# YuHang-max/3DSAD-main

Measured on AMD Instinct MI355X. Metric: scenes/sec (16384-pt KITTI-shaped) through SA+cluster path, higher is better.
Workload: dtype f32

## Files before the change

### 3dsad-main_amd/csrc/mlp_layer.hip

```cpp
#include "common.h"
#include <map>
#include <mutex>
#include <utility>

namespace {

#include "reg_common.h"

constexpr int LWAVES = 4;
constexpr int SLOTS = 16;

using sad::LayerJob;
using sad::LayerMulti;

constexpr int KC = 2;
constexpr int STAGE_F4 = KC * 8 * 64;

__device__ __forceinline__ int job_rows(const LayerJob &jb) { return jb.rowtab ? jb.rowtab[0] : jb.rows; }

struct RowInfo {
    int q, grp;
    bool live, whole;
    unsigned xoff;
    float4 rel;
};
template <bool GATHER>
__device__ __forceinline__ RowInfo row_info(const LayerJob &jb, int rt, int lane, bool need_gid) {
    RowInfo r;
    const int j = lane & 31, h = lane >> 5;
    const int total = job_rows(jb);
    r.q = rt * 32 + j;
    r.live = r.q < total;
    if (!r.live) r.q = total - 1;
    int src = r.q, gv = 0;
    if (GATHER || need_gid) gv = jb.row_gid[r.q];
    if (GATHER) src = jb.row_src[r.q];
    r.grp = gv & (WHOLE_BIT - 1);
    r.whole = (gv & WHOLE_BIT) != 0;
    r.xoff = (unsigned)src * (unsigned)jb.ldx * 4u;
    r.rel = make_float4(0.f, 0.f, 0.f, 0.f);
    if (GATHER && h == 0) {
        const float *pq = jb.xyz + (long long)src * 3;
        const float *pc = jb.new_xyz + (long long)r.grp * 3;
        r.rel = make_float4(pq[0] - pc[0], pq[1] - pc[1], pq[2] - pc[2], 0.f);
    }
    return r;
}

struct Chunk { float4 a0, a1, a2, a3, b0, b1, b2, b3; };
static_assert(KC == 4 || KC == 2, "Chunk holds up to four activation fragments");

template <bool GATHER>
__device__ __forceinline__ Chunk load_chunk_of(const LayerJob &jb, const unsigned xoff, const int ob, const int c, const int wave, const int lane) {
    const int h = lane >> 5;
    const int KG = jb.kg;
    const char *xb = reinterpret_cast<const char *>(jb.x);
    const float4 *wf = reinterpret_cast<const float4 *>(jb.packed + jb.off + jb.np) + (size_t)(ob * 4) * KG * 64;
    const unsigned ulane = (unsigned)lane;
    float4 ga[4], gb[KC];
#pragma unroll
    for (int i = 0; i < KC; ++i) {
        const int f = wave * KC + i;
        const int gk = c * KC + (f >> 2);
        ga[i] = (wf + ((size_t)(f & 3) * KG + (gk < KG ? gk : KG - 1)) * 64)[ulane];
    }
#pragma unroll
    for (int u = 0; u < KC; ++u) {
        int g = c * KC + u;
        g = g < KG ? g : KG - 1;
        if constexpr (GATHER) {
            const int ch = 2 * g - 1 + h;
            const int cc = ch < 0 ? 0 : (ch < jb.cpr ? ch : jb.cpr - 1);
            gb[u] = *reinterpret_cast<const float4 *>(xb + (size_t)(xoff + 16u * (unsigned)cc));
        } else {
            gb[u] = *reinterpret_cast<const float4 *>((xb + (size_t)g * 32) + (size_t)(xoff + 16u * (unsigned)h));
        }
    }
    return Chunk{ga[0], ga[1], ga[KC > 2 ? 2 : 0], ga[KC > 2 ? 3 : 0], gb[0], gb[1], gb[KC > 2 ? 2 : 0], gb[KC > 2 ? 3 : 0]};
}

struct Prefetched {
    Chunk ck;
    float4 rel;
    unsigned xoff;
    int valid;
    int next;
};
struct NextItem {
    int ji;
    int rb, ob;
};
struct NextSource {
    int dyn;
    int pulled;
    int stat;
    int own;
};
constexpr int META_ITEM = 0, META_I0 = 1, META_N = 2;

template <bool GATHER, bool LAST>
__device__ __forceinline__ Prefetched gemm_item(const LayerMulti &lm, const LayerJob &jb, const int rb, const int ob, float4 *lds,
                                                const Prefetched pin, const NextSource ns) {
    Prefetched pre;
    pre.valid = 0;
    pre.next = 0x7FFFFFFF;
    int *meta = reinterpret_cast<int *>(lds + 2 * STAGE_F4);
    auto publish_next = [&]() {
        if (ns.dyn && threadIdx.x == 0) meta[META_ITEM] = ns.pulled * 8 + ns.own;
    };
    const int tid = threadIdx.x, lane = tid & 63, wave = __builtin_amdgcn_readfirstlane(tid >> 6);
    const int h = lane >> 5;
    const int wy = wave >> 1, wx = wave & 1;
    const int KG = jb.kg;
    const int NC = (KG + KC - 1) / KC;
    unsigned fr_xoff;
    float4 fr_rel;
    if (pin.valid) {
        fr_xoff = pin.xoff;
        fr_rel = pin.rel;
    } else {
        const RowInfo fr = row_info<GATHER>(jb, rb * 4 + wave, lane, false);
        fr_xoff = fr.xoff;
        fr_rel = fr.rel;
    }
    auto load_chunk = [&](int c) -> Chunk { return load_chunk_of<GATHER>(jb, fr_xoff, ob, c, wave, lane); };
    auto store_chunk = [&](const Chunk ck, int c, float4 *st) {
        const float4 ga[4] = {ck.a0, ck.a1, ck.a2, ck.a3}, gb[4] = {ck.b0, ck.b1, ck.b2, ck.b3};
#pragma unroll
        for (int i = 0; i < KC; ++i) {
            const int f = wave * KC + i;
            st[((f >> 2) * 8 + (f & 3)) * 64 + lane] = ga[i];
        }
#pragma unroll
        for (int u = 0; u < KC; ++u) {
            const int g = c * KC + u;
            float4 v = gb[u];
            if constexpr (GATHER) {
                const int ch = 2 * g - 1 + h;
                const bool ok = ch >= 0 && ch < jb.cpr;
                v.x = ok ? v.x : 0.f; v.y = ok ? v.y : 0.f; v.z = ok ? v.z : 0.f; v.w = ok ? v.w : 0.f;
                const bool first = g == 0 && h == 0;
                v.x = first ? fr_rel.x : v.x; v.y = first ? fr_rel.y : v.y; v.z = first ? fr_rel.z : v.z; v.w = first ? fr_rel.w : v.w;
            }
            if (g >= KG) v = make_float4(0.f, 0.f, 0.f, 0.f);
            float ops[4];
            to_operands(v.x, v.y, v.z, v.w, ops);
            st[(u * 8 + 4 + wave) * 64 + lane] = make_float4(ops[0], ops[1], ops[2], ops[3]);
        }
    };
    f32x16 acc[2][2];
    {
        const float *bias = jb.packed + jb.off + (ob * 4 + 2 * wx) * 32;
#pragma unroll
        for (int oc = 0; oc < 2; ++oc)
#pragma unroll
            for (int a = 0; a < 4; ++a) {
                const float4 bv = *reinterpret_cast<const float4 *>(bias + oc * 32 + 8 * a + 4 * h);
#pragma unroll
                for (int rt = 0; rt < 2; ++rt) {
                    acc[rt][oc][4 * a + 0] = bv.x; acc[rt][oc][4 * a + 1] = bv.y; acc[rt][oc][4 * a + 2] = bv.z; acc[rt][oc][4 * a + 3] = bv.w;
                }
            }
    }
    __syncthreads();
    Chunk nxt;
    if (pin.valid) nxt = pin.ck;
    else nxt = load_chunk(0);
    store_chunk(nxt, 0, lds);
    if (NC == 1) publish_next();
    __syncthreads();
#pragma unroll 1
    for (int c = 0; c < NC; ++c) {
        float4 *cur = lds + (c & 1) * STAGE_F4;
        if (c + 1 < NC) {
            nxt = load_chunk(c + 1);
        } else {
          const int nitem = __builtin_amdgcn_readfirstlane(ns.dyn ? meta[META_ITEM] : ns.stat);
          const int mi0 = __builtin_amdgcn_readfirstlane(meta[META_I0]);
          pre.next = nitem;
          if (nitem < __builtin_amdgcn_readfirstlane(meta[META_N])) {
            const int nji = nitem < mi0 ? 0 : 1;
            const int nit = nitem - (nji ? mi0 : 0);
            const int nnog = nji ? lm.j[1].nog : lm.j[0].nog;
            NextItem nx;
            nx.ji = nji;
            nx.rb = nit / nnog;
            nx.ob = nit % nnog;
#define SAD_FETCH_NEXT(NJ)                                                                         \
    do {                                                                                           \
        if ((NJ).gather) {                                                                         \
            const RowInfo nf = row_info<true>((NJ), nx.rb * 4 + wave, lane, false);                \
            pre.xoff = nf.xoff;                                                                    \
            pre.rel = nf.rel;                                                                      \
            pre.ck = load_chunk_of<true>((NJ), nf.xoff, nx.ob, 0, wave, lane);                     \
        } else {                                                                                   \
            const RowInfo nf = row_info<false>((NJ), nx.rb * 4 + wave, lane, false);               \
            pre.xoff = nf.xoff;                                                                    \
            pre.rel = nf.rel;                                                                      \
            pre.ck = load_chunk_of<false>((NJ), nf.xoff, nx.ob, 0, wave, lane);                    \
        }                                                                                          \
    } while (0)
            if (nx.ji == 0) SAD_FETCH_NEXT(lm.j[0]);
            else SAD_FETCH_NEXT(lm.j[1]);
#undef SAD_FETCH_NEXT
            pre.valid = 1;
          }
        }
        float4 wa[2][2], xa[2][2];
#pragma unroll
        for (int i = 0; i < 2; ++i) {
            wa[0][i] = cur[(0 * 8 + 2 * wx + i) * 64 + lane];
            xa[0][i] = cur[(0 * 8 + 4 + 2 * wy + i) * 64 + lane];
        }
#pragma unroll
        for (int u = 0; u < KC; ++u) {
            if (u + 1 < KC) {
#pragma unroll
                for (int i = 0; i < 2; ++i) {
                    wa[(u + 1) & 1][i] = cur[((u + 1) * 8 + 2 * wx + i) * 64 + lane];
                    xa[(u + 1) & 1][i] = cur[((u + 1) * 8 + 4 + 2 * wy + i) * 64 + lane];
                }
            }
            __builtin_amdgcn_sched_barrier(0);
#pragma unroll
            for (int rt = 0; rt < 2; ++rt) {
                const float ops[4] = {xa[u & 1][rt].x, xa[u & 1][rt].y, xa[u & 1][rt].z, xa[u & 1][rt].w};
#pragma unroll
                for (int oc = 0; oc < 2; ++oc) acc[rt][oc] = mma4(acc[rt][oc], wa[u & 1][oc], ops);
            }
            __builtin_amdgcn_sched_barrier(0);
        }
        if (c + 1 < NC) store_chunk(nxt, c + 1, lds + ((c + 1) & 1) * STAGE_F4);
        if (c + 2 == NC) publish_next();
        __syncthreads();
    }
    if (jb.relu) {
#pragma unroll
        for (int rt = 0; rt < 2; ++rt)
#pragma unroll
            for (int oc = 0; oc < 2; ++oc)
#pragma unroll
                for (int g = 0; g < 16; ++g) acc[rt][oc][g] = acc[rt][oc][g] > 0.f ? acc[rt][oc][g] : 0.f;
    }
#pragma unroll
    for (int rt = 0; rt < 2; ++rt) {
        const RowInfo ri = row_info<false>(jb, rb * 4 + 2 * wy + rt, lane, LAST);
        const int j = lane & 31;
        if constexpr (!LAST) {
            if (ri.live) {
                float *yrow = jb.y + (long long)ri.q * jb.ldy + (ob * 4 + 2 * wx) * 32 + 4 * h;
#pragma unroll
                for (int oc = 0; oc < 2; ++oc)
#pragma unroll
                    for (int a = 0; a < 4; ++a)
                        *reinterpret_cast<float4 *>(yrow + oc * 32 + 8 * a) =
                            make_float4(acc[rt][oc][4 * a], acc[rt][oc][4 * a + 1], acc[rt][oc][4 * a + 2], acc[rt][oc][4 * a + 3]);
            }
        } else {
            float *stage = reinterpret_cast<float *>(lds) + wave * (SLOTS * 64);
            const int key = ri.live ? ri.grp + 1 : 0;
            const PoolMasks pm = pool_masks(key);
            const int nkey = __shfl_down(key, 1, 64), pkey = __shfl_up(key, 1, 64);
            const bool tail = ri.live && (j == 31 || nkey != key);
            const bool head = ri.live && (j == 0 || pkey != key);
            const unsigned heads = (unsigned)__ballot(head), tails = (unsigned)__ballot(tail);
            const int ngroups = __builtin_popcount(heads);
            const int slot = __builtin_popcount(heads & (0xFFFFFFFFu >> (31 - j))) - 1;
            const bool staged = ngroups <= SLOTS;
            const int ch0 = (ob * 4 + 2 * wx) * 32;
#pragma unroll
            for (int oc = 0; oc < 2; ++oc) {
                const f32x16 t = seg_max16(acc[rt][oc], pm);
                if (!tail) continue;
                if (staged) {
                    float *d = stage + slot * 64 + oc * 32 + 4 * h;
#pragma unroll
                    for (int a = 0; a < 4; ++a) *reinterpret_cast<float4 *>(d + 8 * a) = make_float4(t[4 * a], t[4 * a + 1], t[4 * a + 2], t[4 * a + 3]);
                } else {
                    float *o = jb.out + (long long)ri.grp * jb.ld_out + jb.col_off + ch0 + oc * 32 + 4 * h;
#pragma unroll
                    for (int a = 0; a < 4; ++a)
#pragma unroll
                        for (int e = 0; e < 4; ++e) {
                            if (ch0 + oc * 32 + 8 * a + 4 * h + e >= jb.cout_last) continue;
                            if (ri.whole) o[8 * a + e] = t[4 * a + e];
                            else atomic_max_pos(o + 8 * a + e, t[4 * a + e]);
                        }
                }
            }
            if (staged) {
                unsigned rem = tails;
                for (int s = 0; s < ngroups; ++s) {
                    const int p = __builtin_ctz(rem);
                    rem &= rem - 1;
                    const int g = __builtin_amdgcn_readlane(ri.grp, p);
                    const bool w = __builtin_amdgcn_readlane((int)ri.whole, p) != 0;
                    float *orow = jb.out + (long long)g * jb.ld_out + jb.col_off + ch0;
                    const float *sp = stage + s * 64;
                    if (ch0 + lane < jb.cout_last) {
                        if (w) orow[lane] = sp[lane];
                        else atomic_max_pos(orow + lane, sp[lane]);
                    }
                }
            }
        }
    }
    return pre;
}

__global__ __launch_bounds__(LWAVES * 64) __attribute__((amdgpu_waves_per_eu(2, 2))) void mlp_layer_kernel(const LayerMulti lm) {
    extern __shared__ __attribute__((aligned(16))) float4 lds4[];
    int *meta = reinterpret_cast<int *>(lds4 + 2 * STAGE_F4);
    const int i0 = ((job_rows(lm.j[0]) + 127) / 128) * lm.j[0].nog;
    const int nitems = lm.n > 1 ? i0 + ((job_rows(lm.j[1]) + 127) / 128) * lm.j[1].nog : i0;
    const int dyn = lm.queue != nullptr;
    const sad::ItemQueue Q = sad::itemq_init(lm.queue, dyn ? 8 : 0);
    int item = blockIdx.x;
    if (threadIdx.x == 0) {
        meta[META_I0] = i0;
        meta[META_N] = nitems;
        if (dyn) meta[META_ITEM] = sad::itemq_item(Q, Q.own, sad::itemq_pull(Q));
    }
    __syncthreads();
    if (dyn) item = meta[META_ITEM];
    Prefetched pre;
    pre.valid = 0;
    while (true) {
        if (item >= nitems) {
            if (!dyn) break;
            __syncthreads();
            if (threadIdx.x == 0) meta[META_ITEM] = sad::itemq_steal(Q, nitems);
            __syncthreads();
            item = meta[META_ITEM];
            if (item >= nitems) break;
            pre.valid = 0;
        }
        const int ji = item < i0 ? 0 : 1;
        const int it = item - (ji ? i0 : 0);
        const LayerJob &jb = lm.j[ji];
        const int nog = jb.nog;
        NextSource ns;
        ns.dyn = dyn;
        ns.pulled = 0;
        if (dyn && threadIdx.x == 0) ns.pulled = sad::itemq_pull(Q);
        ns.stat = item + (int)gridDim.x;
        ns.own = Q.own;
        if (jb.gather) {
            if (jb.last) pre = gemm_item<true, true>(lm, jb, it / nog, it % nog, lds4, pre, ns);
            else pre = gemm_item<true, false>(lm, jb, it / nog, it % nog, lds4, pre, ns);
        } else {
            if (jb.last) pre = gemm_item<false, true>(lm, jb, it / nog, it % nog, lds4, pre, ns);
            else pre = gemm_item<false, false>(lm, jb, it / nog, it % nog, lds4, pre, ns);
        }
        item = pre.next;
    }
    if (dyn && threadIdx.x == 0) sad::itemq_done(Q, (int)gridDim.x);
}

}

namespace sad {

int *stream_item_queue(hipStream_t st) {
    static std::mutex mu;
    static std::map<std::pair<int, hipStream_t>, int *> queues;
    hipStreamCaptureStatus cap = hipStreamCaptureStatusNone;
    if (hipStreamIsCapturing(st, &cap) != hipSuccess || cap != hipStreamCaptureStatusNone) {
        (void)hipGetLastError();
        return nullptr;
    }
    int dev = 0;
    if (hipGetDevice(&dev) != hipSuccess) {
        (void)hipGetLastError();
        return nullptr;
    }
    std::lock_guard<std::mutex> lk(mu);
    auto it = queues.find({dev, st});
    if (it != queues.end()) return it->second;
    int *q = nullptr;
    if (hipMalloc(&q, sizeof(int) * ITEMQ_INTS) != hipSuccess) {
        (void)hipGetLastError();
        return nullptr;
    }
    if (hipMemsetAsync(q, 0, sizeof(int) * ITEMQ_INTS, st) != hipSuccess) {
        (void)hipGetLastError();
        (void)hipFree(q);
        return nullptr;
    }
    queues[{dev, st}] = q;
    return q;
}

int launch_layers(const LayerMulti &lm_in, long long max_items, hipStream_t st) {
    LayerMulti lm = lm_in;
    lm.queue = get_option(OPT_MLP_LAYER_QUEUE) == 1 ? stream_item_queue(st) : nullptr;
    static std::atomic<uint64_t> attr_done{0};
    lds_attr_once(attr_done, reinterpret_cast<const void *>(&mlp_layer_kernel), 160 * 1024);
    const size_t lds = sizeof(float4) * ((size_t)2 * STAGE_F4 + 1);
    static std::atomic<int> per_cu{0};
    int pc = per_cu.load(std::memory_order_relaxed);
    if (pc == 0) {
        int nb = 0;
        if (hipOccupancyMaxActiveBlocksPerMultiprocessor(&nb, mlp_layer_kernel, LWAVES * 64, lds) != hipSuccess || nb < 1) {
            (void)hipGetLastError();
            nb = 2;
        }
        pc = nb > 2 ? 2 : nb;
        per_cu.store(pc, std::memory_order_relaxed);
    }
    if (get_option(OPT_MLP_DYN_SLOTS) > 0 && get_option(OPT_MLP_DYN_SLOTS) < pc) pc = get_option(OPT_MLP_DYN_SLOTS);
    const int cus = sad::device_cus();
    long long grid = (long long)cus * pc;
    const long long cap = max_items;
    if (grid > cap) grid = cap < 1 ? 1 : cap;
    hipLaunchKernelGGL(mlp_layer_kernel, dim3((unsigned)grid), dim3(LWAVES * 64), lds, st, lm);
    return check_launch("sad_mlp_chain_f32 (layer-streamed chain)");
}

}
```

### 3dsad-main_amd/csrc/reg_common.h

```cpp
#pragma once
#include "prims.h"

constexpr int WHOLE_BIT = 1 << 30;
using sad::RegChain;
using sad::RegMulti;

struct Swapped { float lo, hi; };
__device__ __forceinline__ Swapped swap32(float a, float b) {
    const auto r = __builtin_amdgcn_permlane32_swap(__builtin_bit_cast(unsigned, a), __builtin_bit_cast(unsigned, b), false, false);
    const unsigned r0 = r[0], r1 = r[1];
    return {__builtin_bit_cast(float, r0), __builtin_bit_cast(float, r1)};
}

__device__ __forceinline__ void to_operands(float v0, float v1, float v2, float v3, float *out) {
    const Swapped s01 = swap32(v0, v1);
    const Swapped s23 = swap32(v2, v3);
    out[0] = s01.lo;
    out[1] = s23.lo;
    out[2] = s01.hi;
    out[3] = s23.hi;
}

__device__ __forceinline__ f32x16 mma4(f32x16 acc, const float4 a, const float *b) {
    acc = __builtin_amdgcn_mfma_f32_32x32x2f32(a.x, b[0], acc, 0, 0, 0);
    acc = __builtin_amdgcn_mfma_f32_32x32x2f32(a.y, b[1], acc, 0, 0, 0);
    acc = __builtin_amdgcn_mfma_f32_32x32x2f32(a.z, b[2], acc, 0, 0, 0);
    acc = __builtin_amdgcn_mfma_f32_32x32x2f32(a.w, b[3], acc, 0, 0, 0);
    return acc;
}

__device__ __forceinline__ f32x16 bias_tile(const float *sb, int h) {
    f32x16 t;
#pragma unroll
    for (int a = 0; a < 4; ++a) {
        const float4 bv = *reinterpret_cast<const float4 *>(sb + 8 * a + 4 * h);
        t[4 * a + 0] = bv.x; t[4 * a + 1] = bv.y; t[4 * a + 2] = bv.z; t[4 * a + 3] = bv.w;
    }
    return t;
}

__device__ __forceinline__ f32x16 relu16(f32x16 t) {
#pragma unroll
    for (int g = 0; g < 16; ++g) t[g] = __builtin_amdgcn_fmed3f(t[g], 0.f, __builtin_inff());
    return t;
}

template <int CTRL, int ROWMASK>
__device__ __forceinline__ int dpp_i(int v) {
    return __builtin_amdgcn_update_dpp(0, v, CTRL, ROWMASK, 0xF, true);
}

struct PoolMasks {
    bool m[5];
    bool any[5];
};

__device__ __forceinline__ PoolMasks pool_masks(int key) {
    PoolMasks pm;
    pm.m[0] = dpp_i<0x111, 0xF>(key) == key;
    pm.m[1] = dpp_i<0x112, 0xF>(key) == key;
    pm.m[2] = dpp_i<0x114, 0xF>(key) == key;
    pm.m[3] = dpp_i<0x118, 0xF>(key) == key;
    pm.m[4] = dpp_i<0x142, 0xA>(key) == key;
#pragma unroll
    for (int k = 0; k < 5; ++k) pm.any[k] = __ballot(pm.m[k]) != 0;
    return pm;
}

__device__ __forceinline__ f32x16 seg_max16(f32x16 t, const PoolMasks &pm) {
    unsigned x[16];
#pragma unroll
    for (int g = 0; g < 16; ++g) {
        const float f = t[g];
        x[g] = __builtin_bit_cast(unsigned, f);
    }
#define SAD_STEP(CTRL, RM, K)                                                   \
    if (pm.any[K]) {                                                            \
        _Pragma("unroll") for (int g = 0; g < 16; ++g) {                        \
            const unsigned u = (unsigned)dpp_i<CTRL, RM>((int)x[g]);            \
            const unsigned r = u > x[g] ? u : x[g];                             \
            x[g] = pm.m[K] ? r : x[g];                                          \
        }                                                                       \
    }
    SAD_STEP(0x111, 0xF, 0)
    SAD_STEP(0x112, 0xF, 1)
    SAD_STEP(0x114, 0xF, 2)
    SAD_STEP(0x118, 0xF, 3)
    SAD_STEP(0x142, 0xA, 4)
#undef SAD_STEP
#pragma unroll
    for (int g = 0; g < 16; ++g) t[g] = __builtin_bit_cast(float, x[g]);
    return t;
}

__device__ __forceinline__ void pool_store(f32x16 t, const PoolMasks &pm, bool tail, bool whole, float *orow, int o, int h,
                                           const RegChain &c) {
    t = seg_max16(t, pm);
    if (tail) {
#pragma unroll
        for (int a = 0; a < 4; ++a) {
            const int ch = o * 32 + 8 * a + 4 * h;
            if (whole && c.vec_out && ch + 3 < c.cout_last) {
                *reinterpret_cast<float4 *>(orow + ch) = make_float4(t[4 * a], t[4 * a + 1], t[4 * a + 2], t[4 * a + 3]);
            } else {
#pragma unroll
                for (int e = 0; e < 4; ++e) {
                    if (ch + e >= c.cout_last) continue;
                    if (whole) orow[ch + e] = t[4 * a + e];
                    else atomic_max_pos(orow + ch + e, t[4 * a + e]);
                }
            }
        }
    }
}

struct Stage {
    float *lds;
    int slot;
    unsigned tails;
    int ngroups;
};

template <int COUT>
__device__ __forceinline__ void pool_stage(f32x16 t, const PoolMasks &pm, bool tail, const Stage &sg, int o, int h) {
    t = seg_max16(t, pm);
    if (tail) {
        float *d = sg.lds + sg.slot * COUT + o * 32 + 4 * h;
#pragma unroll
        for (int a = 0; a < 4; ++a)
            *reinterpret_cast<float4 *>(d + 8 * a) = make_float4(t[4 * a], t[4 * a + 1], t[4 * a + 2], t[4 * a + 3]);
    }
}

template <int COUT>
__device__ __forceinline__ void stage_flush(const Stage &sg, int grp, bool whole, int lane, const RegChain &c) {
    unsigned rem = sg.tails;
    for (int s = 0; s < sg.ngroups; ++s) {
        const int p = __builtin_ctz(rem);
        rem &= rem - 1;
        const int g = __builtin_amdgcn_readlane(grp, p);
        const bool w = __builtin_amdgcn_readlane((int)whole, p) != 0;
        float *orow = c.out + (long long)g * c.ld_out + c.col_off;
        const float *src = sg.lds + s * COUT;
        if (w && c.vec_out && COUT == c.cout_last) {
            if (lane * 4 < COUT) *reinterpret_cast<float4 *>(orow + lane * 4) = *reinterpret_cast<const float4 *>(src + lane * 4);
        } else {
#pragma unroll
            for (int k = 0; k < (COUT + 63) / 64; ++k) {
                const int ch = lane + 64 * k;
                if (ch < COUT && ch < c.cout_last) {
                    if (w) orow[ch] = src[ch];
                    else atomic_max_pos(orow + ch, src[ch]);
                }
            }
        }
    }
}
```

Measured before the change: 8553.

## Transpose last-layer MFMA so rows lie in registers and pool via in-register scan

For the last MLP layer, the MFMA operand order is swapped so each lane holds one output channel and the accumulator registers hold rows. The segmented max-pool then becomes a register-level scan over rows, using permlane32 swaps, instead of DPP cross-lane masks plus LDS staging. Results are emitted per segment tail with coalesced per-channel stores or atomics. This removes the LDS staging buffer and its flush loop, and the DPP segmented-max passes. In exchange it adds a serial 16-step scan, per-row readlane and emit branches, and scalar (non-vector) stores.

Measured after the change: 8447. 0.988x the previous value.

```diff
diff --git a/3dsad-main_amd/csrc/mlp_layer.hip b/3dsad-main_amd/csrc/mlp_layer.hip
--- a/3dsad-main_amd/csrc/mlp_layer.hip
+++ b/3dsad-main_amd/csrc/mlp_layer.hip
@@ -8,7 +8,6 @@
 #include "reg_common.h"
 
 constexpr int LWAVES = 4;
-constexpr int SLOTS = 16;
 
 using sad::LayerJob;
 using sad::LayerMulti;
@@ -19,7 +18,7 @@
 __device__ __forceinline__ int job_rows(const LayerJob &jb) { return jb.rowtab ? jb.rowtab[0] : jb.rows; }
 
 struct RowInfo {
-    int q, grp;
+    int q, grp, gv;
     bool live, whole;
     unsigned xoff;
     float4 rel;
@@ -35,6 +34,7 @@
     int src = r.q, gv = 0;
     if (GATHER || need_gid) gv = jb.row_gid[r.q];
     if (GATHER) src = jb.row_src[r.q];
+    r.gv = gv;
     r.grp = gv & (WHOLE_BIT - 1);
     r.whole = (gv & WHOLE_BIT) != 0;
     r.xoff = (unsigned)src * (unsigned)jb.ldx * 4u;
@@ -149,7 +149,17 @@
         }
     };
     f32x16 acc[2][2];
-    {
+    if constexpr (LAST) {
+        const float *bias = jb.packed + jb.off + (ob * 4 + 2 * wx) * 32 + (lane & 31);
+#pragma unroll
+        for (int oc = 0; oc < 2; ++oc) {
+            const float bv = bias[oc * 32];
+#pragma unroll
+            for (int rt = 0; rt < 2; ++rt)
+#pragma unroll
+                for (int g = 0; g < 16; ++g) acc[rt][oc][g] = bv;
+        }
+    } else {
         const float *bias = jb.packed + jb.off + (ob * 4 + 2 * wx) * 32;
 #pragma unroll
         for (int oc = 0; oc < 2; ++oc)
@@ -226,7 +236,10 @@
             for (int rt = 0; rt < 2; ++rt) {
                 const float ops[4] = {xa[u & 1][rt].x, xa[u & 1][rt].y, xa[u & 1][rt].z, xa[u & 1][rt].w};
 #pragma unroll
-                for (int oc = 0; oc < 2; ++oc) acc[rt][oc] = mma4(acc[rt][oc], wa[u & 1][oc], ops);
+                for (int oc = 0; oc < 2; ++oc) {
+                    if constexpr (LAST) acc[rt][oc] = mma4_rows(acc[rt][oc], ops, wa[u & 1][oc]);
+                    else acc[rt][oc] = mma4(acc[rt][oc], wa[u & 1][oc], ops);
+                }
             }
             __builtin_amdgcn_sched_barrier(0);
         }
@@ -239,8 +252,7 @@
         for (int rt = 0; rt < 2; ++rt)
 #pragma unroll
             for (int oc = 0; oc < 2; ++oc)
-#pragma unroll
-                for (int g = 0; g < 16; ++g) acc[rt][oc][g] = acc[rt][oc][g] > 0.f ? acc[rt][oc][g] : 0.f;
+                acc[rt][oc] = relu16(acc[rt][oc]);
     }
 #pragma unroll
     for (int rt = 0; rt < 2; ++rt) {
@@ -257,52 +269,21 @@
                             make_float4(acc[rt][oc][4 * a], acc[rt][oc][4 * a + 1], acc[rt][oc][4 * a + 2], acc[rt][oc][4 * a + 3]);
             }
         } else {
-            float *stage = reinterpret_cast<float *>(lds) + wave * (SLOTS * 64);
-            const int key = ri.live ? ri.grp + 1 : 0;
-            const PoolMasks pm = pool_masks(key);
-            const int nkey = __shfl_down(key, 1, 64), pkey = __shfl_up(key, 1, 64);
-            const bool tail = ri.live && (j == 31 || nkey != key);
-            const bool head = ri.live && (j == 0 || pkey != key);
-            const unsigned heads = (unsigned)__ballot(head), tails = (unsigned)__ballot(tail);
-            const int ngroups = __builtin_popcount(heads);
-            const int slot = __builtin_popcount(heads & (0xFFFFFFFFu >> (31 - j))) - 1;
-            const bool staged = ngroups <= SLOTS;
-            const int ch0 = (ob * 4 + 2 * wx) * 32;
-#pragma unroll
-            for (int oc = 0; oc < 2; ++oc) {
-                const f32x16 t = seg_max16(acc[rt][oc], pm);
-                if (!tail) continue;
-                if (staged) {
-                    float *d = stage + slot * 64 + oc * 32 + 4 * h;
-#pragma unroll
-                    for (int a = 0; a < 4; ++a) *reinterpret_cast<float4 *>(d + 8 * a) = make_float4(t[4 * a], t[4 * a + 1], t[4 * a + 2], t[4 * a + 3]);
-                } else {
-                    float *o = jb.out + (long long)ri.grp * jb.ld_out + jb.col_off + ch0 + oc * 32 + 4 * h;
-#pragma unroll
-                    for (int a = 0; a < 4; ++a)
-#pragma unroll
-                        for (int e = 0; e < 4; ++e) {
-                            if (ch0 + oc * 32 + 8 * a + 4 * h + e >= jb.cout_last) continue;
-                            if (ri.whole) o[8 * a + e] = t[4 * a + e];
-                            else atomic_max_pos(o + 8 * a + e, t[4 * a + e]);
-                        }
+            const RowSegs sg = row_segs(ri.live ? ri.grp + 1 : 0, j);
+            unsigned carry[2];
+            rows_scan<2>(acc[rt], carry, sg, h);
+            const int ld_out = __builtin_amdgcn_readfirstlane(jb.ld_out), cout_last = __builtin_amdgcn_readfirstlane(jb.cout_last);
+            const int ch = (ob * 4 + 2 * wx) * 32 + j;
+            float *const o0 = jb.out + jb.col_off + ch;
+            rows_emit<2>(acc[rt], carry, sg, ri.gv, h, [&](int gv, const float (&v)[2]) {
+                float *o = o0 + (long long)(gv & (WHOLE_BIT - 1)) * ld_out;
+#pragma unroll
+                for (int oc = 0; oc < 2; ++oc) {
+                    if (ch + oc * 32 >= cout_last) continue;
+                    if (gv & WHOLE_BIT) o[oc * 32] = v[oc];
+                    else atomic_max_pos(o + oc * 32, v[oc]);
                 }
-            }
-            if (staged) {
-                unsigned rem = tails;
-                for (int s = 0; s < ngroups; ++s) {
-                    const int p = __builtin_ctz(rem);
-                    rem &= rem - 1;
-                    const int g = __builtin_amdgcn_readlane(ri.grp, p);
-                    const bool w = __builtin_amdgcn_readlane((int)ri.whole, p) != 0;
-                    float *orow = jb.out + (long long)g * jb.ld_out + jb.col_off + ch0;
-                    const float *sp = stage + s * 64;
-                    if (ch0 + lane < jb.cout_last) {
-                        if (w) orow[lane] = sp[lane];
-                        else atomic_max_pos(orow + lane, sp[lane]);
-                    }
-                }
-            }
+            });
         }
     }
     return pre;
diff --git a/3dsad-main_amd/csrc/reg_common.h b/3dsad-main_amd/csrc/reg_common.h
--- a/3dsad-main_amd/csrc/reg_common.h
+++ b/3dsad-main_amd/csrc/reg_common.h
@@ -29,6 +29,14 @@
     return acc;
 }
 
+__device__ __forceinline__ f32x16 mma4_rows(f32x16 acc, const float *x, const float4 w) {
+    acc = __builtin_amdgcn_mfma_f32_32x32x2f32(x[0], w.x, acc, 0, 0, 0);
+    acc = __builtin_amdgcn_mfma_f32_32x32x2f32(x[1], w.y, acc, 0, 0, 0);
+    acc = __builtin_amdgcn_mfma_f32_32x32x2f32(x[2], w.z, acc, 0, 0, 0);
+    acc = __builtin_amdgcn_mfma_f32_32x32x2f32(x[3], w.w, acc, 0, 0, 0);
+    return acc;
+}
+
 __device__ __forceinline__ f32x16 bias_tile(const float *sb, int h) {
     f32x16 t;
 #pragma unroll
@@ -91,6 +99,86 @@
 #pragma unroll
     for (int g = 0; g < 16; ++g) t[g] = __builtin_bit_cast(float, x[g]);
     return t;
+}
+
+struct RowSegs {
+    unsigned heads;
+    unsigned tails;
+};
+
+__device__ __forceinline__ RowSegs row_segs(int key, int j) {
+    const int nkey = __shfl_down(key, 1, 64), pkey = __shfl_up(key, 1, 64);
+    const bool live = key != 0;
+    const bool tail = live && (j == 31 || nkey != key);
+    const bool head = !live || j == 0 || pkey != key;
+    return RowSegs{(unsigned)__ballot(head), (unsigned)__ballot(tail)};
+}
+
+__device__ __forceinline__ bool half_lanes(unsigned lo, unsigned hi) {
+    return __builtin_amdgcn_inverse_ballot_w64((lo ? 0xFFFFFFFFull : 0ull) | (hi ? 0xFFFFFFFF00000000ull : 0ull));
+}
+
+__device__ __forceinline__ constexpr int row_reg(int r) { return (r & 3) + 4 * (r >> 3) + 8 * ((r >> 2) & 1); }
+
+template <int N>
+__device__ __forceinline__ void rows_scan(f32x16 (&t)[N], unsigned (&carry)[N], const RowSegs sg, int h) {
+    unsigned x[N][16];
+#pragma unroll
+    for (int n = 0; n < N; ++n) {
+#pragma unroll
+        for (int g = 0; g < 16; ++g) {
+            const float f = t[n][g];
+            x[n][g] = __builtin_bit_cast(unsigned, f);
+        }
+#pragma unroll
+        for (int e = 0; e < 8; ++e) {
+            const auto r = __builtin_amdgcn_permlane32_swap(x[n][e], x[n][e + 8], false, false);
+            const unsigned r0 = r[0], r1 = r[1];
+            x[n][e] = r0;
+            x[n][e + 8] = r1;
+        }
+    }
+#pragma unroll
+    for (int r = 1; r < 16; ++r) {
+        const bool head = half_lanes((sg.heads >> r) & 1u, (sg.heads >> (r + 16)) & 1u);
+#pragma unroll
+        for (int n = 0; n < N; ++n) {
+            const unsigned y = x[n][row_reg(r - 1)], v = x[n][row_reg(r)];
+            const unsigned m = y > v ? y : v;
+            x[n][row_reg(r)] = head ? v : m;
+        }
+    }
+    const bool carries = half_lanes(0u, !((sg.heads >> 16) & 1u));
+#pragma unroll
+    for (int n = 0; n < N; ++n) {
+        const unsigned y = x[n][row_reg(15)];
+        const auto c = __builtin_amdgcn_permlane32_swap(y, y, false, false);
+        const unsigned c0 = c[0];
+        carry[n] = carries ? c0 : 0u;
+#pragma unroll
+        for (int g = 0; g < 16; ++g) t[n][g] = __builtin_bit_cast(float, x[n][g]);
+    }
+}
+
+template <int N, class Emit>
+__device__ __forceinline__ void rows_emit(const f32x16 (&t)[N], const unsigned (&carry)[N], const RowSegs sg, int gv, int h, Emit emit) {
+    const unsigned up = sg.tails >> 16;
+    const int carried = (up && !((sg.heads >> 16) & 1u)) ? __builtin_ctz(up) : -1;
+#pragma unroll
+    for (int r = 0; r < 16; ++r) {
+        const unsigned t0 = (sg.tails >> r) & 1u, t1 = (sg.tails >> (r + 16)) & 1u;
+        if (!(t0 | t1)) continue;
+        const int g0 = __builtin_amdgcn_readlane(gv, r), g1 = __builtin_amdgcn_readlane(gv, r + 16);
+        float v[N];
+#pragma unroll
+        for (int n = 0; n < N; ++n) {
+            const float f = t[n][row_reg(r)];
+            unsigned u = __builtin_bit_cast(unsigned, f);
+            if (r == carried) u = u > carry[n] ? u : carry[n];
+            v[n] = __builtin_bit_cast(float, u);
+        }
+        if (half_lanes(t0, t1)) emit(h ? g1 : g0, v);
+    }
 }
 
 __device__ __forceinline__ void pool_store(f32x16 t, const PoolMasks &pm, bool tail, bool whole, float *orow, int o, int h,
```
